# firechecking/CleanTransformer

Measured on AMD Instinct MI355X. Metric: SFT tokens/sec/step Bloom-560M bf16, higher is better.
Workload: dtype bf16

## Files before the change

cleantransformer_amd/_lib.py:

```python
from __future__ import annotations

import ctypes as C
import os

import torch

from ._build import LIB_PATH as _DEFAULT_LIB_PATH

LIB_PATH = os.environ.get("CTMI_LIB_PATH") or _DEFAULT_LIB_PATH

F32, BF16, F16 = 0, 1, 2
OPT_LEGACY_GRID = 4
OPT_SHADOW_F16 = 2
EPI_NONE, EPI_GELU, EPI_DGELU, EPI_RELU, EPI_DRELU, EPI_GELUG, EPI_MUL = 0, 1, 2, 3, 4, 5, 6
MT_MAX = 24
PROF_CLASSES = ("gemm_fwd", "gemm_dgrad", "gemm_wgrad", "lm_head", "attn_fwd", "attn_bwd", "layernorm", "loss", "optimizer", "reduce", "other")
ABI_VERSION = 15

vp, i64, i32, f32 = C.c_void_p, C.c_int64, C.c_int, C.c_float


class CtmiError(RuntimeError):
    pass


class AttnDesc(C.Structure):
    _fields_ = [(n, i64) for n in ("B", "nh", "Sq", "Sk", "hd",
                                   "q_bs", "q_hs", "q_rs", "k_bs", "k_hs", "k_rs",
                                   "v_bs", "v_hs", "v_rs", "o_bs", "o_hs", "o_rs",
                                   "am_b", "am_h", "am_q", "am_k")] + [("scale", f32), ("causal", i32), ("future_fill", f32), ("dropout_seed", C.c_uint32), ("dropout_p", f32), ("reserved_", i32)]


# ... 60 lines not shown
    "ctmi_ddp_all_gather": (C.c_int, [C.c_void_p, C.c_void_p, C.c_void_p, C.c_int64, C.c_void_p]),
    "ctmi_ddp_broadcast": (C.c_int, [C.c_void_p, C.c_void_p, C.c_int64, C.c_int, C.c_void_p]),
    "ctmi_ddp_wait": (C.c_int, [C.c_void_p, C.c_void_p]),
    "ctmi_dropout_hash": (C.c_uint32, [C.c_uint32]),
    "ctmi_dropout_keep_hash": (C.c_uint32, [C.c_uint32, C.c_uint32]),
    "ctmi_dropout_threshold": (C.c_uint32, [f32]),
    "ctmi_dropout": (i32, [vp, vp, vp, i64, f32, C.c_uint32, i32, vp]),
    "ctmi_adamw_step": (i32, [C.POINTER(vp), C.POINTER(vp), C.POINTER(vp), C.POINTER(vp), C.POINTER(vp), C.POINTER(i64),
                              i32, f32, f32, f32, f32, f32, i32, i32, i32, f32, vp]),
    "ctmi_adamw_set_hyper": (i32, [vp, f32, f32, f32, f32, f32, i32, i32, i32, f32, vp]),
    "ctmi_adamw_step_dev": (i32, [C.POINTER(vp), C.POINTER(vp), C.POINTER(vp), C.POINTER(vp), C.POINTER(vp), C.POINTER(i64), i32, vp, vp]),
    "ctmi_sgd_step": (i32, [C.POINTER(vp), C.POINTER(vp), C.POINTER(vp), C.POINTER(vp), C.POINTER(i64),
                            i32, f32, f32, f32, f32, i32, vp]),
    "ctmi_cast": (i32, [vp, i32, vp, i32, i64, vp]),
    "ctmi_transpose_cast": (i32, [vp, vp, i32, i64, i64, vp]),
    "ctmi_sumsq": (i32, [vp, i64, vp, i32, vp]),
    "ctmi_scale": (i32, [vp, i64, f32, vp, vp]),
    "ctmi_scale_copy": (i32, [vp, vp, i64, f32, vp]),
    "ctmi_amp_unscale": (i32, [C.POINTER(vp), C.POINTER(i64), i32, vp, vp]),
    "ctmi_amp_update": (i32, [vp, f32, f32, i32, vp]),
    "ctmi_argmax": (i32, [vp, i64, vp, i64, i64, i32, vp]),
    "ctmi_row_lse": (i32, [vp, i64, vp, i64, i64, i32, vp]),
    "ctmi_group_topk": (i32, [vp, i64, vp, vp, f32, vp, vp, i64, i32, i64, i32, i32, vp]),
    "ctmi_scores_filter": (i32, [vp, i64, f32, vp, i64, f32, vp, i64, i64, i64, vp]),
    "ctmi_probe": (i32, [i32, vp, vp, vp]),
    "ctmi_clock_probe": (i32, [i32, vp, vp]),
    "ctmi_probe_dyn_lds": (i32, [i64, vp, vp]),
    "ctmi_profile_begin": (i32, []),
    "ctmi_profile_end": (i32, [C.POINTER(f32), C.POINTER(i32)]),
}
# ... 38 lines not shown
```

cleantransformer_amd/csrc/elementwise.hip:

```cpp
#include "common.h"
#include "reduce_jobs.h"
#include "prof.h"
#include <hip/amd_detail/amd_hip_unsafe_atomics.h>

#ifndef CTMI_LN_BWD_PREFETCH
#define CTMI_LN_BWD_PREFETCH 1
#endif

static thread_local char g_err[512] = "";
void ctmi_set_error(const char* fmt, ...) {
    va_list ap; va_start(ap, fmt); vsnprintf(g_err, sizeof(g_err), fmt, ap); va_end(ap);
}
extern "C" const char* ctmi_last_error(void) { return g_err; }
static thread_local bool g_attr_err = false;
void ctmi_dyn_lds(const void* kern, size_t lds_bytes) {
    const hipError_t e = hipFuncSetAttribute(kern, hipFuncAttributeMaxDynamicSharedMemorySize, (int)lds_bytes);
    if (e != hipSuccess) {
        (void)hipGetLastError();
        ctmi_set_error("hipFuncSetAttribute(MaxDynamicSharedMemorySize = %zu bytes) refused: %s", lds_bytes, hipGetErrorString(e));
        g_attr_err = true;
    }
}
bool ctmi_take_attr_error() { const bool r = g_attr_err; g_attr_err = false; return r; }
extern "C" int ctmi_abi_version(void) { return CTMI_ABI_VERSION; }
// ... 1551 lines not shown
        if (c < C && r < R) dst[c * R + r] = Cvt<TD>::from_f(tile[tx][i]);
    }
}
extern "C" int ctmi_transpose_cast(const float* src, void* dst, int dst_dtype, int64_t rows, int64_t cols, void* stream) {
    ProfScope prof__(CTMI_PROF_OTHER, as_stream(stream));
    CTMI_REQUIRE(src && dst && rows > 0 && cols > 0, "transpose_cast: bad args");
    const dim3 grid((unsigned)cdiv64(cols, 64), (unsigned)cdiv64(rows, 64));
    if (dst_dtype == CTMI_F32) hipLaunchKernelGGL((transpose_cast_k<float>), grid, dim3(256), 0, as_stream(stream), src, (float*)dst, rows, cols);
    else if (dst_dtype == CTMI_BF16) hipLaunchKernelGGL((transpose_cast_k<bf16_t>), grid, dim3(256), 0, as_stream(stream), src, (bf16_t*)dst, rows, cols);
    else if (dst_dtype == CTMI_F16) hipLaunchKernelGGL((transpose_cast_k<f16_t>), grid, dim3(256), 0, as_stream(stream), src, (f16_t*)dst, rows, cols);
    else { ctmi_set_error("transpose_cast: unsupported dtype %d", dst_dtype); return CTMI_ERR_UNSUPPORTED; }
    CTMI_CHECK_LAUNCH("transpose_cast");
    return CTMI_OK;
}

__global__ __launch_bounds__(256) void sumsq_k(const float* __restrict__ x, int64_t n, double* __restrict__ out) {
    double s = 0.0;
    for (int64_t i = (int64_t)blockIdx.x * 256 + threadIdx.x; i < n; i += (int64_t)gridDim.x * 256) { const double v = x[i]; s += v * v; }
    for (int o = 32; o > 0; o >>= 1) s += __shfl_xor(s, o, 64);
    __shared__ double sm[4];
    if ((threadIdx.x & 63) == 0) sm[threadIdx.x >> 6] = s;
    __syncthreads();
    if (threadIdx.x == 0) atomicAdd(out, sm[0] + sm[1] + sm[2] + sm[3]);
}
extern "C" int ctmi_sumsq(const float* x, int64_t n, double* out, int accumulate, void* stream) {
    ProfScope prof__(CTMI_PROF_OTHER, as_stream(stream));
    CTMI_REQUIRE(x && out && n >= 0, "sumsq: bad args");
    hipStream_t st = as_stream(stream);
    if (!accumulate) { if (hipMemsetAsync(out, 0, sizeof(double), st) != hipSuccess) { ctmi_set_error("sumsq: memset failed"); return CTMI_ERR_LAUNCH; } }
    if (n == 0) return CTMI_OK;
// ... 203 lines not shown
```

cleantransformer_amd/csrc/gemm.hip:

```cpp
#include "common.h"
#include "reduce_jobs.h"
#include <type_traits>
#include "mma.h"
#include "prof.h"
#include <atomic>
#ifndef CTMI_GEMM_PART
#define CTMI_GEMM_PART (-1)
#endif
#ifndef CTMI_GELU_AUX_WT
#define CTMI_GELU_AUX_WT 0
#endif
#ifndef CTMI_SIDE_PRE8
#define CTMI_SIDE_PRE8 1
#endif
#define CTMI_GEMM_HAS(p) (CTMI_GEMM_PART == -1 || CTMI_GEMM_PART == (p))

constexpr bool glds_k2(bool pp, int wm) { return pp && wm == 4; }
constexpr int glds_ring(bool pp, int wm, bool xlane = false) { return !pp ? 3 : (glds_k2(pp, wm) ? 6 : 4); }
constexpr int glds_patch_bytes(bool pp, int wm, bool xlane = false) { return (pp && !xlane && wm != 4) ? 4 * 8192 : 0; }


template <typename T> struct Tile;
template <> struct Tile<bf16_t> { static constexpr int BM = 128, BN = 128, BK = 64, PADK = 8, PADR = 8; };
template <> struct Tile<f16_t>  { static constexpr int BM = 128, BN = 128, BK = 64, PADK = 8, PADR = 8; };
// ... 345 lines not shown
            const int r = r16 + i;
            const int cpp = g ^ swz4((r >> 2) & 3);
            return *reinterpret_cast<const short8*>(tile + r * 64 + cpp * 16);
        } else {
            const int k = g * 8 + (i >> 2);
            const int b32 = r16 >> 4;
            const int b32s = (b32 & ~7) | ((b32 ^ kkey(k)) & 7);
            const bf16_t* p = reinterpret_cast<const bf16_t*>(tile + k * ROWB + b32s * 32 + 8 * (i & 3));
            const uint2 lo = lds_read_tr_b16(p);
            const uint2 hi = lds_read_tr_b16(p + 4 * ROWS);
            return __builtin_bit_cast(short8, make_uint4(lo.x, lo.y, hi.x, hi.y));
        }
    }
};

template <typename TO, bool AK, bool BKM, int EPI, int WM, int WGN, bool PP, bool RES, bool XLANE, bool GRP, typename GA, typename TE = bf16_t, bool BSUM = false>
__device__ __forceinline__ void glds_body(const GA g) {
    using T = TE;
    static_assert(!GRP || (PP && WM == 4 && WGN == 4 && AK && BKM && EPI == CTMI_EPI_NONE && sizeof(TO) == 4), "grouped launches: weight gradients on the 128x256 ping-pong tile");
    constexpr int NW = 2 * WGN;
    constexpr int BM = WM * 32, BN = WGN * 64, BK = 32, NST = glds_ring(PP, WM, XLANE);
    using TA = GTile<AK, BM>;
    using TB = GTile<BKM, BN>;
    constexpr int STAGE = TA::BYTES + TB::BYTES;
    constexpr int AOFF = 0, BOFF = NST * TA::BYTES;
    constexpr int PA = TA::NINSTR / NW, PB = TB::NINSTR / NW;
    constexpr int LOADS = PA + PB;
    static_assert(PP ? (LOADS == 3 || LOADS == 4) : (LOADS == 4 || LOADS == 6), "vmcnt immediates below assume these DMA piece counts");
    constexpr bool K2 = glds_k2(PP, WM);
    constexpr int FILL = K2 ? NST - 2 : NST - 1;
    constexpr int LAND = K2 ? 2 : 1;
    extern __shared__ __attribute__((aligned(16))) unsigned char smem_raw[];

    const int tiles_m = (int)((g.M + BM - 1) / BM);
    const int tiles_n = (int)((g.N + BN - 1) / BN);
    const int ntile = tiles_m * tiles_n;
    int nwork_;
    if constexpr (GRP) nwork_ = g.nitems; else nwork_ = ntile * g.splits;
    const int nwork = nwork_;
    const int bid = blockIdx.x, G = gridDim.x;
    constexpr int GM = (WM == 8) ? ((AK && BKM) ? 1 : 4) : 8;
    auto decode = [&](int w, int64_t& m0, int64_t& n0, int& split) {
        const int xcd = w & 7, q = nwork >> 3, r8 = nwork & 7;
        const int vid_all = (xcd < r8 ? xcd * (q + 1) : r8 * (q + 1) + (xcd - r8) * q) + (w >> 3);
        split = vid_all / ntile;
        const int vid = vid_all - split * ntile;
        const int group = vid / (GM * tiles_n), first_m = group * GM;
        const int gm = min(GM, tiles_m - first_m);
        const int in_group = vid - group * GM * tiles_n;
        m0 = (int64_t)(first_m + in_group % gm) * BM;
        n0 = (int64_t)(in_group / gm) * BN;
    };

    const int tid = threadIdx.x, lane = tid & 63, lane_ = lane;
    const int wid = __builtin_amdgcn_readfirstlane(tid >> 6);
    const int wr = wid / WGN, wc = wid % WGN;
// ... 103 lines not shown
                st_wt16(d, f32x4{a0, a1, a2, a3});
                st_wt16(d + 4, f32x4{b0, b1, b2, b3});
            }
        if (gs.cs_on) {
            if ((lane >> 4) == 0) {
                float* d = (part ? P.cspart + (half1 ? P.csn : 0) : P.cs) + mw + arow(0) + lane;
                *d = gs.accs[0];
            }
        }
        if constexpr (BSUM) {
            if (gs.csb_on && (lane & 15) == 0) {
                float* d = (part ? P.cspart + (half1 ? P.csn : 0) : P.cs) + nw + (lane >> 4) * 4;
#pragma unroll
                for (int j = 0; j < 4; ++j) *reinterpret_cast<f32x4*>(d + j * 16) = gs.accb[j];
            }
        }
        return;
    }
    if (g.splits > 1) {
        float* S = g.slabs + (int64_t)split * g.M * g.N;
#pragma unroll
        for (int i = 0; i < WM; ++i) {
            const int64_t m = m0 + wr * (WM * 16) + i * 16 + (lane & 15);
            if (m >= g.M) continue;
#pragma unroll
            for (int j = 0; j < 4; ++j) {
                const int64_t n = n0 + wc * 64 + j * 16 + (lane >> 4) * 4;
                if (n >= g.N) continue;
                float v[4] = {acc[i][j][0], acc[i][j][1], acc[i][j][2], acc[i][j][3]};
                if (n + 4 <= g.N && (g.N & 3) == 0) store4<float>(S + m * g.N + n, v);
// ... 400 lines not shown
                    const unsigned char* bs = smem_raw + BOFF + rd * TB::BYTES;
                    short8 af[WM], bf[4];
#pragma unroll
                    for (int j = 0; j < 4; ++j) bf[j] = TB::frag(bs, wc * 64 + j * 16, lane);
#pragma unroll
                    for (int i = 0; i < WM; ++i) af[i] = TA::frag(as, wr * (WM * 16) + arow(i), lane);
                    issue_stage(wrb);
                    wait_stages(FILL - LAND);
                    asm volatile("s_waitcnt lgkmcnt(0)" ::: "memory");
                    __builtin_amdgcn_sched_barrier(0);
                    __builtin_amdgcn_s_barrier();
                    __builtin_amdgcn_sched_barrier(0);
#pragma unroll
                    for (int i = 0; i < WM; ++i)
#pragma unroll
                        for (int j = 0; j < 4; ++j) acc[i][j] = Mma<T>::mma(bf[j], af[i], acc[i][j]);
                    if constexpr (GRP) {
                        if (gs.cs_on) gs.accs = Mma<T>::mma(WG_ONES8, af[0], gs.accs);
                        if constexpr (BSUM) {
                            if (gs.csb_on) {
#pragma unroll
                                for (int j = 0; j < 4; ++j) gs.accb[j] = Mma<T>::mma(bf[j], WG_ONES8, gs.accb[j]);
                            }
                        }
                    }
                    __builtin_amdgcn_sched_barrier(0);
                    __builtin_amdgcn_s_barrier();
                    __builtin_amdgcn_sched_barrier(0);
                    if constexpr ((NST & (NST - 1)) == 0) { rd = (rd + 1) & (NST - 1); wrb = (wrb + 1) & (NST - 1); }
                    else { rd = rd == NST - 1 ? 0 : rd + 1; wrb = wrb == NST - 1 ? 0 : wrb + 1; }
                }
// ... 11 lines not shown
            for (int j = 0; j < 4; ++j) bf[j] = TB::frag(bs, wc * 64 + j * 16, lane);
#pragma unroll
            for (int i = 0; i < WM; ++i) af[i] = TA::frag(as, wr * (WM * 16) + arow(i), lane);
            if (more) {
                issue_stage(wrb);
                stage_issued(); ++inflight; wrb = wrb == NST - 1 ? 0 : wrb + 1;
            }
            wait_stages(inflight - 1 - LAND);
            asm volatile("s_waitcnt lgkmcnt(0)" ::: "memory");
            __builtin_amdgcn_sched_barrier(0);
            __builtin_amdgcn_s_barrier();
            __builtin_amdgcn_sched_barrier(0);
#pragma unroll
            for (int i = 0; i < WM; ++i)
#pragma unroll
                for (int j = 0; j < 4; ++j) acc[i][j] = Mma<T>::mma(bf[j], af[i], acc[i][j]);
            if constexpr (GRP) {
                if (gs.cs_on) gs.accs = Mma<T>::mma(WG_ONES8, af[0], gs.accs);
                if constexpr (BSUM) {
                    if (gs.csb_on) {
#pragma unroll
                        for (int j = 0; j < 4; ++j) gs.accb[j] = Mma<T>::mma(bf[j], WG_ONES8, gs.accb[j]);
                    }
                }
            }
            __builtin_amdgcn_sched_barrier(0);
            __builtin_amdgcn_s_barrier();
            __builtin_amdgcn_sched_barrier(0);
            rd = rd == NST - 1 ? 0 : rd + 1;
            --inflight;
            if (++tc < ntc) continue;
// ... 32 lines not shown
        else asm volatile("s_waitcnt vmcnt(0)" ::: "memory");
        __builtin_amdgcn_s_barrier();
        const bool more = wi < nwork;
        const unsigned char* as = smem_raw + AOFF + rd * TA::BYTES;
        const unsigned char* bs = smem_raw + BOFF + rd * TB::BYTES;
        short8 af[WM], bf[4];
#pragma unroll
        for (int i = 0; i < WM; ++i) af[i] = TA::frag(as, wr * (WM * 16) + arow(i), lane);
#pragma unroll
        for (int j = 0; j < 4; ++j) bf[j] = TB::frag(bs, wc * 64 + j * 16, lane);
        __builtin_amdgcn_s_setprio(1);
#pragma unroll
        for (int i = 0; i < WM; ++i)
#pragma unroll
            for (int j = 0; j < 4; ++j) {
                acc[i][j] = Mma<T>::mma(bf[j], af[i], acc[i][j]);
                const int idx = i * 4 + j;
                if (idx % EVERY == EVERY - 1 && idx / EVERY < LOADS) {
                    if (more) issue_one(wrb, idx / EVERY);
                    __builtin_amdgcn_sched_barrier(0);
                }
            }
        __builtin_amdgcn_s_setprio(0);
        rd = rd == NST - 1 ? 0 : rd + 1;
        --inflight;
        if (more) { stage_issued(); ++inflight; wrb = wrb == NST - 1 ? 0 : wrb + 1; }
        if (++tc < ntc) continue;
        epilogue(m0, n0, split);
        cw += G;
        if (cw >= nwork) break;
        decode(cw, m0, n0, split);
// ... 2 lines not shown
#pragma unroll
        for (int i = 0; i < WM; ++i)
#pragma unroll
            for (int j = 0; j < 4; ++j) acc[i][j] = f32x4{0.f, 0.f, 0.f, 0.f};
    }
}

template <typename TO, bool AK, bool BKM, int EPI, int WM, int WGN, bool PP = false, bool RES = false, bool XLANE = false>
__global__ __launch_bounds__(128 * WGN, 2) void gemm_glds_kernel(GemmArgs g) {
    glds_body<TO, AK, BKM, EPI, WM, WGN, PP, RES, XLANE, false, GemmArgs>(g);
}
template <typename TO, bool AK, bool BKM, int EPI, int WM, int WGN, bool PP = false, bool RES = false, bool XLANE = false>
__global__ __launch_bounds__(128 * WGN, 2) void gemm_glds_kernel_f16(GemmArgs g) {
    glds_body<TO, AK, BKM, EPI, WM, WGN, PP, RES, XLANE, false, GemmArgs, f16_t>(g);
}
#if CTMI_GEMM_HAS(3) || CTMI_GEMM_PART == 8
__global__ __launch_bounds__(512, 2) void gemm_wgrad_grouped_kernel(GroupedArgs g) {
    glds_body<float, true, true, CTMI_EPI_NONE, 4, 4, true, false, false, true, GroupedArgs>(g);
}
__global__ __launch_bounds__(512, 2) void gemm_wgrad_grouped_kernel_f16(GroupedArgs g) {
    glds_body<float, true, true, CTMI_EPI_NONE, 4, 4, true, false, false, true, GroupedArgs, f16_t>(g);
}
__global__ __launch_bounds__(512, 2) void gemm_wgrad_grouped_bsum_kernel(GroupedArgs g) {
    glds_body<float, true, true, CTMI_EPI_NONE, 4, 4, true, false, false, true, GroupedArgs, bf16_t, true>(g);
}
__global__ __launch_bounds__(512, 2) void gemm_wgrad_grouped_bsum_kernel_f16(GroupedArgs g) {
    glds_body<float, true, true, CTMI_EPI_NONE, 4, 4, true, false, false, true, GroupedArgs, f16_t, true>(g);
}
struct WgReduceArgs { GroupProb p[WG_MAXP]; const int4* tiles; int ntiles; };
__global__ __launch_bounds__(256) void wgrad_partials_reduce_k(WgReduceArgs z);
// ... 53 lines not shown
    static int persist_ksteps = -1;
    if (persist_ksteps < 0) { const char* e = getenv("CTMI_GEMM_PERSIST_KSTEPS"); persist_ksteps = e ? atoi(e) : 128; }
    const bool long_tiles = persist_ksteps > 0 && g.k_per_split / 32 > persist_ksteps;
    const unsigned grid = (unsigned)((persist && !long_tiles && nwork > slots) ? slots : nwork);
    if constexpr (std::is_same<TE, f16_t>::value) {
        auto kern = &gemm_glds_kernel_f16<TO, AK, BKM, EPI, WM, WGN, PP, RES, XLANE>;
        ctmi_dyn_lds(reinterpret_cast<const void*>(kern), lds);
        hipLaunchKernelGGL(kern, dim3(grid), dim3(128 * WGN), lds, st, g);
    } else {
        auto kern = &gemm_glds_kernel<TO, AK, BKM, EPI, WM, WGN, PP, RES, XLANE>;
        ctmi_dyn_lds(reinterpret_cast<const void*>(kern), lds);
        hipLaunchKernelGGL(kern, dim3(grid), dim3(128 * WGN), lds, st, g);
    }
}

#if CTMI_GEMM_HAS(0)
std::atomic<int> g_ctmi_policy_shared{-1}, g_ctmi_policy_reserve{-1};
#else
extern std::atomic<int> g_ctmi_policy_shared, g_ctmi_policy_reserve;
#endif
static int shared_level() {
    int v = g_ctmi_policy_shared.load(std::memory_order_relaxed);
    if (v < 0) { const char* e = getenv("CTMI_GEMM_SHARED"); v = e ? std::max(0, std::min(2, atoi(e))) : 0; g_ctmi_policy_shared.store(v, std::memory_order_relaxed); }
    return v;
}
static bool shared_mode() { return shared_level() >= 1; }
static bool shared_tiles() { return shared_level() == 1; }
static int reserved_cus() {
    int v = g_ctmi_policy_reserve.load(std::memory_order_relaxed);
    if (v < 0) { const char* e = getenv("CTMI_GEMM_RESERVE_CUS"); v = e ? std::max(0, std::min(128, atoi(e))) : 0; g_ctmi_policy_reserve.store(v, std::memory_order_relaxed); }
// ... 137 lines not shown
    if (g.splits > 1) {
        const int64_t total = g.M * g.N;
        const unsigned rg = (unsigned)std::min<int64_t>(cdiv64(total, 256), 4096);
        hipLaunchKernelGGL((splitk_reduce<TO>), dim3(rg), dim3(256), 0, st, g.slabs, reinterpret_cast<TO*>(g.C), g.ldc, g.M, g.N, g.splits, g.alpha, g.beta);
        CTMI_CHECK_LAUNCH("gemm_splitk_reduce");
    }
    return CTMI_OK;
}

int ctmi_gemm_bf16_nt(GemmArgs& g, int epi, bool fast, hipStream_t st);
int ctmi_gemm_bf16_nn(GemmArgs& g, int epi, bool fast, hipStream_t st);
int ctmi_gemm_bf16_tn(GemmArgs& g, int epi, bool fast, hipStream_t st);
int ctmi_gemm_f16_nt(GemmArgs& g, int epi, bool fast, hipStream_t st);
int ctmi_gemm_f16_nn(GemmArgs& g, int epi, bool fast, hipStream_t st);
int ctmi_gemm_f16_tn(GemmArgs& g, int epi, bool fast, hipStream_t st);
static int gemm_unsupported(int ak, int bk, int epi, int out_f32) {
    ctmi_set_error("gemm: unsupported combination a_kmajor=%d b_kmajor=%d epilogue=%d out_f32=%d", ak, bk, epi, out_f32);
    return CTMI_ERR_UNSUPPORTED;
}

#if CTMI_GEMM_HAS(1)
int ctmi_gemm_bf16_nt(GemmArgs& g, int epi, bool fast, hipStream_t st) {
    if (epi == CTMI_EPI_NONE) return gemm_launch<bf16_t, bf16_t, false, false, CTMI_EPI_NONE>(g, fast, st);
    if (epi == CTMI_EPI_GELU) return gemm_launch<bf16_t, bf16_t, false, false, CTMI_EPI_GELU>(g, fast, st);
    if (epi == CTMI_EPI_GELUG) return gemm_launch<bf16_t, bf16_t, false, false, CTMI_EPI_GELUG>(g, fast, st);
    if (epi == CTMI_EPI_RELU) return gemm_launch<bf16_t, bf16_t, false, false, CTMI_EPI_RELU>(g, fast, st);
    if (epi == CTMI_EPI_DGELU) return gemm_launch<bf16_t, bf16_t, false, false, CTMI_EPI_DGELU>(g, fast, st);
    return gemm_unsupported(0, 0, epi, 0);
}
#endif
// ... 308 lines not shown
    g.ws = reinterpret_cast<float*>(workspace); g.ws_bytes = workspace_bytes;
    if (workspace != nullptr && epilogue == CTMI_EPI_NONE && bias == nullptr && residual == nullptr && ntile < 384 && K >= 8 * bkt) {
        int64_t want = std::min<int64_t>(8, cdiv64(512, ntile));
        want = std::min<int64_t>(want, K / (4 * bkt));
        want = std::min<int64_t>(want, workspace_bytes / (int64_t)(M * N * sizeof(float)));
        if (want > 1) {
            const int64_t kps = cdiv64(cdiv64(K, want), bkt) * bkt;
            g.splits = (int)cdiv64(K, kps); g.k_per_split = kps; g.slabs = reinterpret_cast<float*>(workspace);
            if (g.splits <= 1) { g.splits = 1; g.k_per_split = K; g.slabs = nullptr; }
        }
    }
    if (dtype == CTMI_F32) return gemm_dispatch_f32(g, a_kmajor, b_kmajor, epilogue, fast, as_stream(stream));
    if (dtype == CTMI_F16) return gemm_dispatch_f16(g, a_kmajor, b_kmajor, epilogue, out_f32, fast, as_stream(stream));
    return gemm_dispatch_bf16(g, a_kmajor, b_kmajor, epilogue, out_f32, fast, as_stream(stream));
}
#endif

#if CTMI_GEMM_PART == 9
#ifndef CTMI_ONE_KERNEL
#define CTMI_ONE_KERNEL bf16_t, false, true, 0, 4, 4, true, false, false
#endif
template __global__ void gemm_glds_kernel<CTMI_ONE_KERNEL>(GemmArgs);
#endif
```

cleantransformer_amd/models/modeling_bloom.py:

```python
from __future__ import annotations

import math
from typing import Optional

import torch

from .. import _lib, ops
from ..generation.generation_util import GenerationMixin
from ..transformer import LayerNorm

Tensor = torch.Tensor


class BloomConfig():

    def __init__(
            self,
            vocab_size=250880,
            hidden_size=64,
            n_layer=2,
            num_attention_heads=8,
            layer_norm_epsilon=1e-5,
            initializer_range=0.02,
            use_cache=True,
# ... 269 lines not shown
    def backward(ctx, dlogits: Tensor):
        h2, weight = ctx.saved_tensors
        B, S, H = ctx.shape
        V = weight.shape[0]
        d2 = dlogits.reshape(B * S, V)
        wc = ops.compute_weight(weight, h2.dtype)
        tie = ctx.tie
        tied = tie is not None and tie.embed_wants
        sync = getattr(weight, "_ct_tied_sync", None) if tied else None
        pre = sync.prescale(weight) if sync is not None else None
        Vp = ops.ZERO_PADDED.pop(d2.data_ptr(), (None, None))[0] if d2.is_cuda else None
        wpad = getattr(weight, "_ct_shadow_pad", None)
        if Vp is not None and d2.stride() == (Vp, 1) and wpad is not None and wpad.shape[0] == Vp and wpad.dtype == h2.dtype:
            dp = d2.as_strided((B * S, Vp), (Vp, 1))
            dh = ops.linear_dgrad(dp, wpad)
            dw = ops.linear_wgrad(dp, h2, alpha=1.0 if pre is None else pre)[:V]
        else:
            d2 = d2 if d2.is_contiguous() else d2.contiguous()
            rows = sync.chunk_rows(V, H) if pre is not None else V
            if rows < V:
                dw = torch.empty((V, H), dtype=torch.float32, device=d2.device)
                sync.announce(tie.n_tokens, d2.device)
                for c0 in range(0, V, rows):
                    c1 = min(V, c0 + rows)
                    ops.gemm(d2[:, c0:], V, True, h2, H, True, c1 - c0, H, B * S, out=dw[c0:c1], out_f32=True, alpha=pre)
                    sync.begin(dw[c0:c1])
                tie.pending, tie.early = dw, sync
                dh = ops.linear_dgrad(d2, wc)
                return dh.view(B, S, H), None, None
            dh = ops.linear_dgrad(d2, wc)
            dw = ops.linear_wgrad(d2, h2, alpha=1.0 if pre is None else pre)
        if tied:
            tie.pending = dw
            if pre is not None:
                sync.announce(tie.n_tokens, dw.device)
                sync.begin(dw)
                tie.early = sync
            dw = None
        return dh.view(B, S, H), dw, None


_FUSED_CE = _os.environ.get("CTMI_FUSED_CE", "1") != "0"


class ShiftedCrossEntropyFn(torch.autograd.Function):

# ... 208 lines not shown
```

cleantransformer_amd/ops.py:

```python
from __future__ import annotations

import contextlib
import os
import ctypes as C
import math
import threading
from typing import Optional, Tuple

import torch

from . import _lib
from ._lib import AttnDesc, BF16, F16, F32, check

Tensor = torch.Tensor


def _p(t: Optional[Tensor]):
    return None if t is None else C.c_void_p(t.data_ptr())


def _stream():
    return C.c_void_p(torch.cuda.current_stream().cuda_stream)


# ... 147 lines not shown
    N = w.shape[0]
    return gemm(x2d, K, False, w, K, False, T, N, K, bias=bias, residual=residual, epilogue=epilogue, aux_out=aux_out, tag=tag, out=out)


def linear_dgrad(dy: Tensor, w: Tensor, epilogue: int = _lib.EPI_NONE, aux_in: Optional[Tensor] = None,
                 residual: Optional[Tensor] = None) -> Tensor:
    T, Nout = dy.shape
    Kin = w.shape[1]
    return gemm(dy, Nout, False, w, Kin, True, T, Kin, Nout, epilogue=epilogue, aux_in=aux_in, residual=residual)


def linear_wgrad(dy: Tensor, x2d: Tensor, out: Optional[Tensor] = None, accumulate: bool = False, alpha: float = 1.0) -> Tensor:
    T, Nout = dy.shape
    Kin = x2d.shape[1]
    return gemm(dy, Nout, True, x2d, Kin, True, Nout, Kin, T, out=out, out_f32=True, beta=int(accumulate), alpha=alpha)


def wgrad_grouped(problems, in_out: bool = False):
    lib = _lib.load()
    arr = (_lib.WgradProblem * len(problems))()
    outs = []
    T = problems[0][0].shape[0]
    for i, (dy, x, want_db) in enumerate(problems):
        _need_cuda(dy, x)
        assert dy.is_contiguous() and x.is_contiguous() and dy.shape[0] == T and x.shape[0] == T
        n_out, n_in = dy.shape[1], x.shape[1]
        dw = torch.empty((n_in, n_out) if in_out else (n_out, n_in), dtype=torch.float32, device=dy.device)
        db = torch.empty(n_out, dtype=torch.float32, device=dy.device) if want_db else None
        arr[i].dy, arr[i].x, arr[i].dw, arr[i].db = dy.data_ptr(), x.data_ptr(), dw.data_ptr(), (None if db is None else db.data_ptr())
        arr[i].n_out, arr[i].n_in, arr[i].in_out = n_out, n_in, int(in_out)
# ... 811 lines not shown
```

include/ctmi355.h:

```cpp
#ifndef CTMI355_H
#define CTMI355_H

#include <stdint.h>

#ifdef __cplusplus
extern "C" {
#endif

#define CTMI_ABI_VERSION 15

enum ctmi_dtype { CTMI_F32 = 0, CTMI_BF16 = 1, CTMI_F16 = 2 };
enum ctmi_status { CTMI_OK = 0, CTMI_ERR_ARG = -1, CTMI_ERR_LAUNCH = -2, CTMI_ERR_UNSUPPORTED = -3 };

int ctmi_abi_version(void);
const char* ctmi_last_error(void);

int ctmi_layernorm_fwd(const void* x, const float* w, const float* b, void* y, float* mean, float* rstd,
                       int64_t rows, int64_t cols, float eps, int dtype, void* stream);
int64_t ctmi_layernorm_bwd_ws(int64_t rows, int64_t cols);
int ctmi_layernorm_bwd(const void* dy, const void* x, const float* w, const float* mean, const float* rstd,
                       const void* dres, void* dx, float* dw, float* db, int accumulate, float* ws,
                       int64_t rows, int64_t cols, int dtype, void* stream);

enum ctmi_epilogue { CTMI_EPI_NONE = 0, CTMI_EPI_GELU = 1, CTMI_EPI_DGELU = 2, CTMI_EPI_RELU = 3, CTMI_EPI_DRELU = 4,
                     CTMI_EPI_GELUG = 5, CTMI_EPI_MUL = 6 };
int ctmi_gemm(const void* A, int64_t lda, int a_kmajor, const void* B, int64_t ldb, int b_kmajor,
              void* C, int64_t ldc, int64_t M, int64_t N, int64_t K,
              float alpha, int beta, const float* bias, const void* residual, int epilogue,
              const void* aux_in, void* aux_out, int out_f32, int dtype,
              void* workspace, int64_t workspace_bytes, void* stream);

typedef struct ctmi_wgrad_problem {
    const void* dy; const void* x;
    float* dw; float* db;
    int64_t n_out, n_in;
    int in_out; int pad_;
} ctmi_wgrad_problem;
int ctmi_wgrad_grouped(const ctmi_wgrad_problem* problems , int count, int64_t T, int dtype,
                       void* workspace , int64_t workspace_bytes, void* stream);

int ctmi_set_launch_policy(int shared, int reserve_cus);
int ctmi_get_launch_policy(int* shared , int* reserve_cus );

enum ctmi_prof_class {
    CTMI_PROF_GEMM_FWD = 0,
// ... 84 lines not shown
                    int decoupled, int mutate_grad, float grad_scale, void* stream);
int ctmi_adamw_set_hyper(void* hyper_dev , float lr, float beta1, float beta2, float eps, float weight_decay,
                         int step, int decoupled, int mutate_grad, float grad_scale, void* stream);
int ctmi_adamw_step_dev(float* const* p , float* const* g , float* const* m , float* const* v ,
                        void* const* shadow , const int64_t* n , int count,
                        const void* hyper_dev , void* stream);
int ctmi_sgd_step(float* const* p, float* const* g, float* const* buf ,
                  void* const* shadow, const int64_t* n, int count, float lr, float momentum, float dampening,
                  float weight_decay, int first_step, void* stream);

int ctmi_amp_unscale(float* const* g , const int64_t* n , int count, float* state , void* stream);
int ctmi_amp_update(float* state , float growth, float backoff, int interval, void* stream);

int ctmi_cast(const void* src, int src_dtype, void* dst, int dst_dtype, int64_t n, void* stream);
int ctmi_transpose_cast(const float* src, void* dst, int dst_dtype, int64_t rows, int64_t cols, void* stream);
int ctmi_sumsq(const float* x, int64_t n, double* out, int accumulate, void* stream);
int ctmi_scale(float* x, int64_t n, float s, const float* s_dev , void* stream);
int ctmi_scale_copy(const float* src, float* dst, int64_t n, float s, void* stream);
int ctmi_argmax(const void* x, int64_t ld, int64_t* out, int64_t rows, int64_t cols, int dtype, void* stream);

int ctmi_row_lse(const void* x, int64_t ld, float* stats , int64_t rows, int64_t cols, int dtype, void* stream);
int ctmi_group_topk(const void* x, int64_t ld, const float* stats, const float* add, float add_mul, float* out_val ,
                    int64_t* out_idx , int64_t groups, int group, int64_t cols, int k, int dtype, void* stream);
int ctmi_scores_filter(const float* x, int64_t ld, float divisor, const float* thr, int64_t thr_stride, float fill, float* out,
                       int64_t ldo, int64_t rows, int64_t cols, void* stream);

#define CTMI_REDUCE_MAX_JOBS 16
typedef struct ctmi_reduce_job {
    const float* src; float* dst; int64_t n; int64_t part_stride; int32_t nparts; int32_t accumulate; float alpha; int32_t pad_;
} ctmi_reduce_job;
// ... 47 lines not shown
```

Measured before the change: 227,400.

## Compute LM-head weight gradient via transposed-activation NN GEMM with transposed store

```diff
diff --git a/cleantransformer_amd/_lib.py b/cleantransformer_amd/_lib.py
--- a/cleantransformer_amd/_lib.py
+++ b/cleantransformer_amd/_lib.py
@@ -15,7 +15,7 @@
 EPI_NONE, EPI_GELU, EPI_DGELU, EPI_RELU, EPI_DRELU, EPI_GELUG, EPI_MUL = 0, 1, 2, 3, 4, 5, 6
 MT_MAX = 24
 PROF_CLASSES = ("gemm_fwd", "gemm_dgrad", "gemm_wgrad", "lm_head", "attn_fwd", "attn_bwd", "layernorm", "loss", "optimizer", "reduce", "other")
-ABI_VERSION = 15
+ABI_VERSION = 16
 
 vp, i64, i32, f32 = C.c_void_p, C.c_int64, C.c_int, C.c_float
 
@@ -106,6 +106,9 @@
                             i32, f32, f32, f32, f32, i32, vp]),
     "ctmi_cast": (i32, [vp, i32, vp, i32, i64, vp]),
     "ctmi_transpose_cast": (i32, [vp, vp, i32, i64, i64, vp]),
+    "ctmi_transpose16": (i32, [vp, i64, vp, i64, i64, i64, i32, vp]),
+    "ctmi_lm_head_wgrad_nn_ok": (i32, [i64, i64, i64, i32]),
+    "ctmi_lm_head_wgrad_nn": (i32, [vp, i64, vp, i64, vp, i64, i64, i64, i64, f32, i32, vp]),
     "ctmi_sumsq": (i32, [vp, i64, vp, i32, vp]),
     "ctmi_scale": (i32, [vp, i64, f32, vp, vp]),
     "ctmi_scale_copy": (i32, [vp, vp, i64, f32, vp]),
diff --git a/cleantransformer_amd/csrc/elementwise.hip b/cleantransformer_amd/csrc/elementwise.hip
--- a/cleantransformer_amd/csrc/elementwise.hip
+++ b/cleantransformer_amd/csrc/elementwise.hip
@@ -1589,6 +1589,44 @@
     return CTMI_OK;
 }
 
+__global__ __launch_bounds__(256) void transpose16_k(const uint16_t* __restrict__ src, int64_t lds_, uint16_t* __restrict__ dst, int64_t ldd, int64_t R, int64_t C) {
+    __shared__ __attribute__((aligned(16))) unsigned char tile[64 * 128];
+    const int64_t r0 = (int64_t)blockIdx.x * 64, c0 = (int64_t)blockIdx.y * 64;
+    const int t = threadIdx.x;
+#pragma unroll
+    for (int h = 0; h < 2; ++h) {
+        const int r = (t >> 3) + 32 * h, cb = t & 7;
+        uint4 v = make_uint4(0u, 0u, 0u, 0u);
+        if (r0 + r < R && c0 + cb * 8 < C) v = *reinterpret_cast<const uint4*>(src + (r0 + r) * lds_ + c0 + cb * 8);
+        *reinterpret_cast<uint4*>(tile + r * 128 + ((cb ^ (r >> 3)) << 4)) = v;
+    }
+    __syncthreads();
+#pragma unroll
+    for (int h = 0; h < 2; ++h) {
+        const int rb = t & 7, c = (t >> 3) + 32 * h;
+        const unsigned char* p = tile + rb * 8 * 128 + (((c >> 3) ^ rb) << 4) + (c & 7) * 2;
+        uint32_t w[4];
+#pragma unroll
+        for (int k = 0; k < 4; ++k) {
+            const uint32_t lo = *reinterpret_cast<const uint16_t*>(p + (2 * k) * 128), hi = *reinterpret_cast<const uint16_t*>(p + (2 * k + 1) * 128);
+            w[k] = lo | (hi << 16);
+        }
+        if (c0 + c < C && r0 + rb * 8 < R) st_wt16(dst + (c0 + c) * ldd + r0 + rb * 8, make_uint4(w[0], w[1], w[2], w[3]));
+    }
+}
+extern "C" int ctmi_transpose16(const void* src, int64_t ld_src, void* dst, int64_t ld_dst, int64_t rows, int64_t cols, int dtype, void* stream) {
+    ProfScope prof__(CTMI_PROF_OTHER, as_stream(stream));
+    CTMI_REQUIRE(src && dst && rows > 0 && cols > 0, "transpose16: bad args");
+    CTMI_REQUIRE(dtype == CTMI_BF16 || dtype == CTMI_F16, "transpose16: 2-byte element types only (dtype %d)", dtype);
+    CTMI_REQUIRE(rows % 8 == 0 && cols % 8 == 0 && ld_src % 8 == 0 && ld_dst % 8 == 0 && ld_src >= cols && ld_dst >= rows, "transpose16: rows, cols and leading dimensions must be multiples of 8");
+    CTMI_REQUIRE(((((uintptr_t)src) | ((uintptr_t)dst)) & 15) == 0, "transpose16: operands must be 16-byte aligned");
+    const dim3 grid((unsigned)cdiv64(rows, 64), (unsigned)cdiv64(cols, 64));
+    CTMI_REQUIRE(grid.y < 65536, "transpose16: too many columns");
+    hipLaunchKernelGGL(transpose16_k, grid, dim3(256), 0, as_stream(stream), (const uint16_t*)src, ld_src, (uint16_t*)dst, ld_dst, rows, cols);
+    CTMI_CHECK_LAUNCH("transpose16");
+    return CTMI_OK;
+}
+
 __global__ __launch_bounds__(256) void sumsq_k(const float* __restrict__ x, int64_t n, double* __restrict__ out) {
     double s = 0.0;
     for (int64_t i = (int64_t)blockIdx.x * 256 + threadIdx.x; i < n; i += (int64_t)gridDim.x * 256) { const double v = x[i]; s += v * v; }
diff --git a/cleantransformer_amd/csrc/gemm.hip b/cleantransformer_amd/csrc/gemm.hip
--- a/cleantransformer_amd/csrc/gemm.hip
+++ b/cleantransformer_amd/csrc/gemm.hip
@@ -383,10 +383,11 @@
     }
 };
 
-template <typename TO, bool AK, bool BKM, int EPI, int WM, int WGN, bool PP, bool RES, bool XLANE, bool GRP, typename GA, typename TE = bf16_t, bool BSUM = false>
+template <typename TO, bool AK, bool BKM, int EPI, int WM, int WGN, bool PP, bool RES, bool XLANE, bool GRP, typename GA, typename TE = bf16_t, bool BSUM = false, bool CT = false>
 __device__ __forceinline__ void glds_body(const GA g) {
     using T = TE;
     static_assert(!GRP || (PP && WM == 4 && WGN == 4 && AK && BKM && EPI == CTMI_EPI_NONE && sizeof(TO) == 4), "grouped launches: weight gradients on the 128x256 ping-pong tile");
+    static_assert(!CT || (PP && WM == 8 && WGN == 4 && !AK && BKM && EPI == CTMI_EPI_NONE && sizeof(TO) == 4 && !RES && !XLANE && !GRP), "transposed store: the fp32 NN product on the 256x256 ping-pong tile");
     constexpr int NW = 2 * WGN;
     constexpr int BM = WM * 32, BN = WGN * 64, BK = 32, NST = glds_ring(PP, WM, XLANE);
     using TA = GTile<AK, BM>;
@@ -408,7 +409,8 @@
     if constexpr (GRP) nwork_ = g.nitems; else nwork_ = ntile * g.splits;
     const int nwork = nwork_;
     const int bid = blockIdx.x, G = gridDim.x;
-    constexpr int GM = (WM == 8) ? ((AK && BKM) ? 1 : 4) : 8;
+    constexpr int GM_C = (WM == 8) ? ((AK && BKM) ? 1 : 4) : 8;
+    const int GM = CT ? tiles_m : GM_C;
     auto decode = [&](int w, int64_t& m0, int64_t& n0, int& split) {
         const int xcd = w & 7, q = nwork >> 3, r8 = nwork & 7;
         const int vid_all = (xcd < r8 ? xcd * (q + 1) : r8 * (q + 1) + (xcd - r8) * q) + (w >> 3);
@@ -542,6 +544,17 @@
 #pragma unroll
                 for (int j = 0; j < 4; ++j) *reinterpret_cast<f32x4*>(d + j * 16) = gs.accb[j];
             }
+        }
+        return;
+    }
+    if constexpr (CT) {
+        float* Cl = reinterpret_cast<float*>(g.C) + m0 + wr * (WM * 16) + (lane >> 4) * 4;
+#pragma unroll
+        for (int j = 0; j < 4; ++j) {
+            const int64_t n = n0 + wc * 64 + j * 16 + (lane & 15);
+            if (n >= g.N) continue;
+#pragma unroll
+            for (int i = 0; i < WM; ++i) st_wt16(Cl + n * g.ldc + i * 16, acc[i][j] * g.alpha);
         }
         return;
     }
@@ -972,7 +985,7 @@
 #pragma unroll
                     for (int i = 0; i < WM; ++i)
 #pragma unroll
-                        for (int j = 0; j < 4; ++j) acc[i][j] = Mma<T>::mma(bf[j], af[i], acc[i][j]);
+                        for (int j = 0; j < 4; ++j) acc[i][j] = CT ? Mma<T>::mma(af[i], bf[j], acc[i][j]) : Mma<T>::mma(bf[j], af[i], acc[i][j]);
                     if constexpr (GRP) {
                         if (gs.cs_on) gs.accs = Mma<T>::mma(WG_ONES8, af[0], gs.accs);
                         if constexpr (BSUM) {
@@ -1014,7 +1027,7 @@
 #pragma unroll
             for (int i = 0; i < WM; ++i)
 #pragma unroll
-                for (int j = 0; j < 4; ++j) acc[i][j] = Mma<T>::mma(bf[j], af[i], acc[i][j]);
+                for (int j = 0; j < 4; ++j) acc[i][j] = CT ? Mma<T>::mma(af[i], bf[j], acc[i][j]) : Mma<T>::mma(bf[j], af[i], acc[i][j]);
             if constexpr (GRP) {
                 if (gs.cs_on) gs.accs = Mma<T>::mma(WG_ONES8, af[0], gs.accs);
                 if constexpr (BSUM) {
@@ -1077,7 +1090,7 @@
         for (int i = 0; i < WM; ++i)
 #pragma unroll
             for (int j = 0; j < 4; ++j) {
-                acc[i][j] = Mma<T>::mma(bf[j], af[i], acc[i][j]);
+                acc[i][j] = CT ? Mma<T>::mma(af[i], bf[j], acc[i][j]) : Mma<T>::mma(bf[j], af[i], acc[i][j]);
                 const int idx = i * 4 + j;
                 if (idx % EVERY == EVERY - 1 && idx / EVERY < LOADS) {
                     if (more) issue_one(wrb, idx / EVERY);
@@ -1110,6 +1123,16 @@
 __global__ __launch_bounds__(128 * WGN, 2) void gemm_glds_kernel_f16(GemmArgs g) {
     glds_body<TO, AK, BKM, EPI, WM, WGN, PP, RES, XLANE, false, GemmArgs, f16_t>(g);
 }
+#if CTMI_GEMM_HAS(2)
+__global__ __launch_bounds__(512, 2) void gemm_glds_ct_kernel(GemmArgs g) {
+    glds_body<float, false, true, CTMI_EPI_NONE, 8, 4, true, false, false, false, GemmArgs, bf16_t, false, true>(g);
+}
+#endif
+#if CTMI_GEMM_HAS(5)
+__global__ __launch_bounds__(512, 2) void gemm_glds_ct_kernel_f16(GemmArgs g) {
+    glds_body<float, false, true, CTMI_EPI_NONE, 8, 4, true, false, false, false, GemmArgs, f16_t, false, true>(g);
+}
+#endif
 #if CTMI_GEMM_HAS(3) || CTMI_GEMM_PART == 8
 __global__ __launch_bounds__(512, 2) void gemm_wgrad_grouped_kernel(GroupedArgs g) {
     glds_body<float, true, true, CTMI_EPI_NONE, 4, 4, true, false, false, true, GroupedArgs>(g);
@@ -1193,6 +1216,25 @@
     }
 }
 
+#if CTMI_GEMM_HAS(2) || CTMI_GEMM_HAS(5)
+template <typename KERN>
+static int glds_ct_launch(KERN kern, GemmArgs& g, hipStream_t st) {
+    const size_t lds = glds_ring(true, 8) * (size_t)(GTile<false, 256>::BYTES + GTile<true, 256>::BYTES) + glds_patch_bytes(true, 8);
+    g.splits = 1; g.k_per_split = g.K; g.slabs = nullptr;
+    const int64_t nwork = cdiv64(g.M, 256) * cdiv64(g.N, 256);
+    ctmi_dyn_lds(reinterpret_cast<const void*>(kern), lds);
+    hipLaunchKernelGGL(kern, dim3((unsigned)nwork), dim3(512), lds, st, g);
+    CTMI_CHECK_LAUNCH("gemm_glds_ct");
+    return CTMI_OK;
+}
+#endif
+#if CTMI_GEMM_HAS(2)
+int ctmi_gemm_bf16_nn_ct(GemmArgs& g, hipStream_t st) { return glds_ct_launch(&gemm_glds_ct_kernel, g, st); }
+#endif
+#if CTMI_GEMM_HAS(5)
+int ctmi_gemm_f16_nn_ct(GemmArgs& g, hipStream_t st) { return glds_ct_launch(&gemm_glds_ct_kernel_f16, g, st); }
+#endif
+
 #if CTMI_GEMM_HAS(0)
 std::atomic<int> g_ctmi_policy_shared{-1}, g_ctmi_policy_reserve{-1};
 #else
@@ -1360,6 +1402,8 @@
 int ctmi_gemm_f16_nt(GemmArgs& g, int epi, bool fast, hipStream_t st);
 int ctmi_gemm_f16_nn(GemmArgs& g, int epi, bool fast, hipStream_t st);
 int ctmi_gemm_f16_tn(GemmArgs& g, int epi, bool fast, hipStream_t st);
+int ctmi_gemm_bf16_nn_ct(GemmArgs& g, hipStream_t st);
+int ctmi_gemm_f16_nn_ct(GemmArgs& g, hipStream_t st);
 static int gemm_unsupported(int ak, int bk, int epi, int out_f32) {
     ctmi_set_error("gemm: unsupported combination a_kmajor=%d b_kmajor=%d epilogue=%d out_f32=%d", ak, bk, epi, out_f32);
     return CTMI_ERR_UNSUPPORTED;
@@ -1698,6 +1742,38 @@
     if (dtype == CTMI_F16) return gemm_dispatch_f16(g, a_kmajor, b_kmajor, epilogue, out_f32, fast, as_stream(stream));
     return gemm_dispatch_bf16(g, a_kmajor, b_kmajor, epilogue, out_f32, fast, as_stream(stream));
 }
+
+static bool lm_head_wgrad_nn_enabled() {
+    static int v = -1;
+    if (v < 0) { const char* e = getenv("CTMI_LMHEAD_WGRAD_NN"); v = (e && e[0] == '0') ? 0 : 1; }
+    return v == 1;
+}
+extern "C" int ctmi_lm_head_wgrad_nn_ok(int64_t V, int64_t H, int64_t T, int dtype) {
+    if (!lm_head_wgrad_nn_enabled() || !glds_enabled()) return 0;
+    if (dtype != CTMI_BF16 && dtype != CTMI_F16) return 0;
+    if (V <= 0 || H <= 0 || T <= 0 || V % 8 != 0 || T % 32 != 0 || H % 256 != 0) return 0;
+    int tile, splits;
+    pick_tile(V, H, T, true, true, CTMI_EPI_NONE, 1, tile, splits);
+    return tile == 3 && splits == 1;
+}
+extern "C" int ctmi_lm_head_wgrad_nn(const void* xt, int64_t ldxt, const void* dy, int64_t lddy, float* dw, int64_t lddw,
+                                     int64_t V, int64_t H, int64_t T, float alpha, int dtype, void* stream) {
+    CTMI_REQUIRE(xt && dy && dw, "lm_head_wgrad_nn: null operand");
+    CTMI_REQUIRE(V > 0 && H > 0 && T > 0 && ldxt >= T && lddy >= V && lddw >= H, "lm_head_wgrad_nn: bad shape V=%lld H=%lld T=%lld", (long long)V, (long long)H, (long long)T);
+    auto al16 = [](const void* p) { return (((uintptr_t)p) & 15) == 0; };
+    if (!ctmi_lm_head_wgrad_nn_ok(V, H, T, dtype) || !al16(xt) || !al16(dy) || !al16(dw) || ldxt % 8 != 0 || lddy % 8 != 0 || lddw % 4 != 0) {
+        ctmi_set_error("lm_head_wgrad_nn: unsupported V=%lld H=%lld T=%lld dtype=%d (or unaligned operands): use ctmi_gemm", (long long)V, (long long)H, (long long)T, dtype);
+        return CTMI_ERR_UNSUPPORTED;
+    }
+    ProfScope prof__(V >= 65536 ? CTMI_PROF_LM_HEAD : CTMI_PROF_GEMM_WGRAD, as_stream(stream));
+    GemmArgs g{};
+    g.A = xt; g.B = dy; g.C = dw; g.lda = ldxt; g.ldb = lddy; g.ldc = lddw; g.M = H; g.N = V; g.K = T;
+    g.alpha = alpha;
+    g.tiles_m = (int)cdiv64(H, 128); g.tiles_n = (int)cdiv64(V, 128);
+    CTMI_REQUIRE((int64_t)g.tiles_m * g.tiles_n < (1LL << 27), "lm_head_wgrad_nn: too many tiles");
+    g.vec_c = 1; g.vec8 = 0;
+    return dtype == CTMI_F16 ? ctmi_gemm_f16_nn_ct(g, as_stream(stream)) : ctmi_gemm_bf16_nn_ct(g, as_stream(stream));
+}
 #endif
 
 #if CTMI_GEMM_PART == 9
diff --git a/cleantransformer_amd/models/modeling_bloom.py b/cleantransformer_amd/models/modeling_bloom.py
--- a/cleantransformer_amd/models/modeling_bloom.py
+++ b/cleantransformer_amd/models/modeling_bloom.py
@@ -307,22 +307,25 @@
         if Vp is not None and d2.stride() == (Vp, 1) and wpad is not None and wpad.shape[0] == Vp and wpad.dtype == h2.dtype:
             dp = d2.as_strided((B * S, Vp), (Vp, 1))
             dh = ops.linear_dgrad(dp, wpad)
-            dw = ops.linear_wgrad(dp, h2, alpha=1.0 if pre is None else pre)[:V]
+            dw = ops.lm_head_wgrad(dp, h2, alpha=1.0 if pre is None else pre)[:V]
         else:
             d2 = d2 if d2.is_contiguous() else d2.contiguous()
             rows = sync.chunk_rows(V, H) if pre is not None else V
             if rows < V:
                 dw = torch.empty((V, H), dtype=torch.float32, device=d2.device)
                 sync.announce(tie.n_tokens, d2.device)
+                xt = None
                 for c0 in range(0, V, rows):
                     c1 = min(V, c0 + rows)
-                    ops.gemm(d2[:, c0:], V, True, h2, H, True, c1 - c0, H, B * S, out=dw[c0:c1], out_f32=True, alpha=pre)
+                    if xt is None and ops.lm_head_wgrad_nn_ok(d2[:, c0:c1], h2):
+                        xt = ops.lm_head_xt(h2)
+                    ops.lm_head_wgrad(d2[:, c0:c1], h2, alpha=pre, out=dw[c0:c1], xt=xt)
                     sync.begin(dw[c0:c1])
                 tie.pending, tie.early = dw, sync
                 dh = ops.linear_dgrad(d2, wc)
                 return dh.view(B, S, H), None, None
             dh = ops.linear_dgrad(d2, wc)
-            dw = ops.linear_wgrad(d2, h2, alpha=1.0 if pre is None else pre)
+            dw = ops.lm_head_wgrad(d2, h2, alpha=1.0 if pre is None else pre)
         if tied:
             tie.pending = dw
             if pre is not None:
diff --git a/cleantransformer_amd/ops.py b/cleantransformer_amd/ops.py
--- a/cleantransformer_amd/ops.py
+++ b/cleantransformer_amd/ops.py
@@ -185,6 +185,46 @@
     T, Nout = dy.shape
     Kin = x2d.shape[1]
     return gemm(dy, Nout, True, x2d, Kin, True, Nout, Kin, T, out=out, out_f32=True, beta=int(accumulate), alpha=alpha)
+
+
+def transpose16(x2d: Tensor, out: Optional[Tensor] = None) -> Tensor:
+    _need_cuda(x2d)
+    R, Cc = x2d.shape
+    assert x2d.stride(1) == 1
+    if out is None:
+        out = torch.empty((Cc, R), dtype=x2d.dtype, device=x2d.device)
+    check(_lib.load().ctmi_transpose16(_p(x2d), x2d.stride(0), _p(out), out.stride(0), R, Cc, dt_code(x2d.dtype), _stream()), "transpose16")
+    return out
+
+
+def lm_head_wgrad_nn_ok(dy: Tensor, x2d: Tensor) -> bool:
+    if not (dy.is_cuda and x2d.is_cuda and dy.dtype == x2d.dtype and dy.dtype in (torch.bfloat16, torch.float16)):
+        return False
+    if dy.stride(1) != 1 or not x2d.is_contiguous() or dy.stride(0) % 8 != 0 or dy.data_ptr() % 16 != 0 or x2d.data_ptr() % 16 != 0:
+        return False
+    T, H = x2d.shape
+    return bool(_lib.load().ctmi_lm_head_wgrad_nn_ok(dy.shape[1], H, T, dt_code(dy.dtype)))
+
+
+def lm_head_xt(x2d: Tensor) -> Tensor:
+    T, H = x2d.shape
+    buf = torch.empty((H, T + 64), dtype=x2d.dtype, device=x2d.device)
+    return transpose16(x2d, out=buf[:, :T])
+
+
+def lm_head_wgrad(dy: Tensor, x2d: Tensor, alpha: float = 1.0, out: Optional[Tensor] = None, xt: Optional[Tensor] = None) -> Tensor:
+    T, V = dy.shape
+    H = x2d.shape[1]
+    out_ok = out is None or (out.dtype == torch.float32 and out.stride(1) == 1 and out.stride(0) % 4 == 0 and out.data_ptr() % 16 == 0)
+    if not (out_ok and lm_head_wgrad_nn_ok(dy, x2d)):
+        return gemm(dy, dy.stride(0), True, x2d, H, True, V, H, T, out=out, out_f32=True, alpha=alpha)
+    if xt is None:
+        xt = lm_head_xt(x2d)
+    if out is None:
+        out = torch.empty((V, H), dtype=torch.float32, device=dy.device)
+    check(_lib.load().ctmi_lm_head_wgrad_nn(_p(xt), xt.stride(0), _p(dy), dy.stride(0), _p(out), out.stride(0), V, H, T, float(alpha), dt_code(dy.dtype),
+                                            _stream()), "lm_head_wgrad_nn")
+    return out
 
 
 def wgrad_grouped(problems, in_out: bool = False):
diff --git a/include/ctmi355.h b/include/ctmi355.h
--- a/include/ctmi355.h
+++ b/include/ctmi355.h
@@ -7,7 +7,7 @@
 extern "C" {
 #endif
 
-#define CTMI_ABI_VERSION 15
+#define CTMI_ABI_VERSION 16
 
 enum ctmi_dtype { CTMI_F32 = 0, CTMI_BF16 = 1, CTMI_F16 = 2 };
 enum ctmi_status { CTMI_OK = 0, CTMI_ERR_ARG = -1, CTMI_ERR_LAUNCH = -2, CTMI_ERR_UNSUPPORTED = -3 };
@@ -29,6 +29,10 @@
               float alpha, int beta, const float* bias, const void* residual, int epilogue,
               const void* aux_in, void* aux_out, int out_f32, int dtype,
               void* workspace, int64_t workspace_bytes, void* stream);
+
+int ctmi_lm_head_wgrad_nn_ok(int64_t V, int64_t H, int64_t T, int dtype);
+int ctmi_lm_head_wgrad_nn(const void* xt, int64_t ldxt, const void* dy, int64_t lddy, float* dw, int64_t lddw,
+                          int64_t V, int64_t H, int64_t T, float alpha, int dtype, void* stream);
 
 typedef struct ctmi_wgrad_problem {
     const void* dy; const void* x;
@@ -143,6 +147,7 @@
 
 int ctmi_cast(const void* src, int src_dtype, void* dst, int dst_dtype, int64_t n, void* stream);
 int ctmi_transpose_cast(const float* src, void* dst, int dst_dtype, int64_t rows, int64_t cols, void* stream);
+int ctmi_transpose16(const void* src, int64_t ld_src, void* dst, int64_t ld_dst, int64_t rows, int64_t cols, int dtype, void* stream);
 int ctmi_sumsq(const float* x, int64_t n, double* out, int accumulate, void* stream);
 int ctmi_scale(float* x, int64_t n, float s, const float* s_dev , void* stream);
 int ctmi_scale_copy(const float* src, float* dst, int64_t n, float s, void* stream);
```

Result: no change. 228,500, median of 6 (+0.5%).
